# declare-lab/tango

Measured on NVIDIA H100. Metric: audio_seconds_per_second, higher is better.
Workload: dtype bf16

## Files before the change

### tango_b200/csrc/attention_tc.cu

```cuda
#include "tng_ptx.cuh"
#include "tng_internal.h"
#include <stdlib.h>

namespace tng {

constexpr int AT_BM = 128;
constexpr int AT_BN = 64;
constexpr int AT_D = 64;
constexpr int AT_QCHUNK = AT_BM * 128;
constexpr int AT_KCHUNK = AT_BN * 128;
constexpr int AT_NB = 3;
constexpr int AT_THREADS = 256;

struct AttnParams {
  int Lq, Lk, heads;
  int q_col0, q_lo_off, k_col0, k_lo_off, v_col0, v_lo_off;
  const float* kbias;
  __nv_bfloat16* out;
  long long ld_o;
  int split_off;
  float scale_log2e;
};

template <int NSPLIT>
struct AttnCfg {
  static constexpr int Q_BYTES = NSPLIT * AT_QCHUNK;
  static constexpr int KV_BYTES = NSPLIT * AT_KCHUNK;
  static constexpr int SMEM_BYTES = Q_BYTES + AT_NB * 2 * KV_BYTES + 128;
};

template <int NSPLIT>
__global__ void __launch_bounds__(AT_THREADS, (NSPLIT == 1) ? 2 : 1)
attention_kernel(const __grid_constant__ CUtensorMap qmap, const __grid_constant__ CUtensorMap kmap,
                 const __grid_constant__ CUtensorMap vmap, const __grid_constant__ AttnParams p) {
  using Cfg = AttnCfg<NSPLIT>;
  extern __shared__ __align__(1024) uint8_t smem[];
  uint8_t* sQ = smem;
  uint8_t* sK = sQ + Cfg::Q_BYTES;
  uint8_t* sV = sK + AT_NB * Cfg::KV_BYTES;
  uint64_t* bars = reinterpret_cast<uint64_t*>(sV + AT_NB * Cfg::KV_BYTES);
  uint64_t* bar_q = bars;
  uint64_t* full_k = bars + 1;
  uint64_t* full_v = bars + 1 + AT_NB;
  uint64_t* empty_k = bars + 1 + 2 * AT_NB;
  uint64_t* empty_v = bars + 1 + 3 * AT_NB;

  const int tid = threadIdx.x;
  const int warp = tid >> 5;
  const int lane = tid & 31;
  const int wg = warp >> 2;
  const int q0 = blockIdx.x * AT_BM;
  const int head = blockIdx.y;
  const int b = blockIdx.z;
  const int n_tiles = (p.Lk + AT_BN - 1) / AT_BN;

  auto load_k = [&](int t) {
    const int buf = t % AT_NB;
    mbar_arrive_expect_tx(&full_k[buf], Cfg::KV_BYTES);
#pragma unroll
    for (int s = 0; s < NSPLIT; ++s)
      tma_load_3d(sK + buf * Cfg::KV_BYTES + s * AT_KCHUNK, &kmap, &full_k[buf], p.k_col0 + s * p.k_lo_off + head * AT_D,
                  t * AT_BN, b);
  };
  auto load_v = [&](int t) {
    const int buf = t % AT_NB;
    mbar_arrive_expect_tx(&full_v[buf], Cfg::KV_BYTES);
#pragma unroll
    for (int s = 0; s < NSPLIT; ++s)
      tma_load_3d(sV + buf * Cfg::KV_BYTES + s * AT_KCHUNK, &vmap, &full_v[buf], p.v_col0 + s * p.v_lo_off + head * AT_D,
                  t * AT_BN, b);
  };

  if (tid == 0) {
    if ((smem_u32(smem) & 1023u) != 0) __trap();
    tma_prefetch_desc(&qmap);
    tma_prefetch_desc(&kmap);
    tma_prefetch_desc(&vmap);
    mbar_init(bar_q, 1);
    for (int i = 0; i < AT_NB; ++i) {
      mbar_init(&full_k[i], 1);
      mbar_init(&full_v[i], 1);
      mbar_init(&empty_k[i], 2);
      mbar_init(&empty_v[i], 2);
    }
    fence_mbar_init();
    mbar_arrive_expect_tx(bar_q, Cfg::Q_BYTES);
#pragma unroll
    for (int s = 0; s < NSPLIT; ++s)
      tma_load_3d(sQ + s * AT_QCHUNK, &qmap, bar_q, p.q_col0 + s * p.q_lo_off + head * AT_D, q0, b);
    for (int t = 0; t < AT_NB && t < n_tiles; ++t) { load_k(t); load_v(t); }
  }
  __syncthreads();

  constexpr int NT = (NSPLIT == 1) ? 1 : 3;
  const int qsel[3] = {0, 1, 0}, ksel[3] = {0, 0, 1};
  const uint32_t q_base = smem_u32(sQ) + wg * (64 * 128);
  const uint32_t k_base = smem_u32(sK), v_base = smem_u32(sV);
  const float sc = p.scale_log2e;
  constexpr float LOG2E = 1.4426950408889634f;
  const float* kb = p.kbias ? p.kbias + static_cast<long long>(b) * p.Lk : nullptr;
  const int t4 = lane & 3;
  float m_run[2] = {-INFINITY, -INFINITY};
  float l_run[2] = {0.f, 0.f};
  float o[32];
#pragma unroll
  for (int i = 0; i < 32; ++i) o[i] = 0.f;

  mbar_wait(bar_q, 0);
  for (int t = 0; t < n_tiles; ++t) {
    const int buf = t % AT_NB;
    const uint32_t ph = (t / AT_NB) & 1;
    if (tid == 0 && t >= 1 && t - 1 + AT_NB < n_tiles) {
      const int pb = (t - 1) % AT_NB;
      const uint32_t pph = ((t - 1) / AT_NB) & 1;
      mbar_wait(&empty_k[pb], pph);
      load_k(t - 1 + AT_NB);
      mbar_wait(&empty_v[pb], pph);
      load_v(t - 1 + AT_NB);
    }
    float s[32];
    mbar_wait(&full_k[buf], ph);
    fence_regs(s);
    wgmma_fence();
#pragma unroll
    for (int u = 0; u < NT; ++u) {
      const uint64_t qd = wgmma_desc_sw128(q_base + qsel[u] * AT_QCHUNK, 16, 1024);
      const uint64_t kd = wgmma_desc_sw128(k_base + buf * Cfg::KV_BYTES + ksel[u] * AT_KCHUNK, 16, 1024);
#pragma unroll
      for (int k = 0; k < AT_D / 16; ++k) wgmma_ss<64>(s, qd + 2 * k, kd + 2 * k, (u > 0 || k > 0) ? 1u : 0u);
    }
    wgmma_commit();
    wgmma_wait<0>();
    fence_regs(s);
    if ((tid & 127) == 0) mbar_arrive(&empty_k[buf]);

    const int kv0 = t * AT_BN;
    const bool tail = (kb != nullptr) || (kv0 + AT_BN > p.Lk);
#pragma unroll
    for (int j = 0; j < 8; ++j) {
#pragma unroll
      for (int e = 0; e < 2; ++e) {
        float bias = 0.f;
        if (tail) {
          const int kv = kv0 + 8 * j + 2 * t4 + e;
          bias = kv < p.Lk ? (kb ? __ldg(kb + kv) * LOG2E : 0.f) : -INFINITY;
        }
        s[4 * j + e] = fmaf(s[4 * j + e], sc, bias);
        s[4 * j + 2 + e] = fmaf(s[4 * j + 2 + e], sc, bias);
      }
    }
    float corr[2];
    softmax_step(s, m_run, l_run, corr);
    rescale_rows(o, corr);
    uint32_t pa[NSPLIT][4][4];
    pack_p(pa[0], s);
    if constexpr (NSPLIT == 2) pack_p<true>(pa[1], s);

    mbar_wait(&full_v[buf], ph);
    fence_regs(o);
    wgmma_fence();
#pragma unroll
    for (int u = 0; u < NT; ++u) {
      const int ps = (NSPLIT == 2 && u == 1) ? NSPLIT - 1 : 0;
      const uint64_t vd = wgmma_desc_sw128(v_base + buf * Cfg::KV_BYTES + ksel[u] * AT_KCHUNK, 1024, 1024);
#pragma unroll
      for (int kk = 0; kk < AT_BN / 16; ++kk) wgmma_rs_n64_tb(o, pa[ps][kk], vd + ((kk * 2048) >> 4), 1u);
    }
    wgmma_commit();
    wgmma_wait<0>();
    fence_regs(o);
    if ((tid & 127) == 0) mbar_arrive(&empty_v[buf]);
  }

  float inv[2];
  softmax_inv(l_run, inv);
#pragma unroll
  for (int h = 0; h < 2; ++h) {
    const int q = q0 + 64 * wg + 16 * (warp & 3) + (lane >> 2) + 8 * h;
    if (q >= p.Lq) continue;
    __nv_bfloat16* op = p.out + (static_cast<long long>(b) * p.Lq + q) * p.ld_o + head * AT_D + 2 * t4;
#pragma unroll
    for (int j = 0; j < 8; ++j) {
      const float y0 = o[4 * j + 2 * h] * inv[h], y1 = o[4 * j + 2 * h + 1] * inv[h];
      *reinterpret_cast<uint32_t*>(op + 8 * j) = pack_bf16(y0, y1);
      if (p.split_off > 0)
        *reinterpret_cast<uint32_t*>(op + p.split_off + 8 * j) = pack_bf16_lo(y0, y1);
    }
  }
}

template <int NSPLIT>
static int launch_attn(const tng_attn_desc* d, const CUtensorMap& qm, const CUtensorMap& km, const CUtensorMap& vm,
                       const AttnParams& p, cudaStream_t st) {
  const int rc = set_max_dynamic_smem<attention_kernel<NSPLIT>>(AttnCfg<NSPLIT>::SMEM_BYTES, "attention");
  if (rc) return rc;
  dim3 grid((d->Lq + AT_BM - 1) / AT_BM, d->heads, d->batch);
  attention_kernel<NSPLIT><<<grid, AT_THREADS, AttnCfg<NSPLIT>::SMEM_BYTES, st>>>(qm, km, vm, p);
  return check_launch("attention");
}

}

using namespace tng;

extern "C" int tng_attention(const tng_attn_desc* d, void* stream) {
  if (!d || !d->q || !d->k || !d->v || !d->out) return set_error(TNG_EINVAL, "attention: null argument");
  if (d->nsplit != 1 && d->nsplit != 2) return set_error(TNG_EINVAL, "attention: nsplit=%d", d->nsplit);
  if (d->batch <= 0 || d->heads <= 0 || d->Lq <= 0 || d->Lk <= 0) return set_error(TNG_EINVAL, "attention: bad sizes");
  if (d->scale <= 0.f) return set_error(TNG_EINVAL, "attention: scale must be positive");
  if (d->ld_o % 8 || d->split_off % 8 || (reinterpret_cast<uintptr_t>(d->out) & 15))
    return set_error(TNG_EINVAL, "attention: output must allow 16-byte stores");
  AttnParams p;
  p.Lq = d->Lq; p.Lk = d->Lk; p.heads = d->heads;
  p.q_col0 = d->q_col0; p.q_lo_off = d->q_lo_off;
  p.k_col0 = d->k_col0; p.k_lo_off = d->k_lo_off;
  p.v_col0 = d->v_col0; p.v_lo_off = d->v_lo_off;
  p.kbias = d->kbias;
  p.out = reinterpret_cast<__nv_bfloat16*>(d->out);
  p.ld_o = d->ld_o; p.split_off = d->split_off;
  p.scale_log2e = d->scale * 1.4426950408889634f;
  CUtensorMap qm, km, vm;
  int rc = encode_tmap_rows_bf16(&qm, d->q, d->ld_q, d->Lq, d->batch, AT_BM);
  if (!rc) rc = encode_tmap_rows_bf16(&km, d->k, d->ld_k, d->Lk, d->batch, AT_BN);
  if (!rc) rc = encode_tmap_rows_bf16(&vm, d->v, d->ld_v, d->Lk, d->batch, AT_BN);
  if (rc) return rc;
  cudaStream_t st = reinterpret_cast<cudaStream_t>(stream);
  if (d->nsplit == 2) return launch_attn<2>(d, qm, km, vm, p, st);
  return launch_attn<1>(d, qm, km, vm, p, st);
}
```

### tango_b200/csrc/tng_ptx.cuh

```cuda
#pragma once
#include <cuda_runtime.h>
#include <cuda_bf16.h>
#include <cuda.h>
#include <stdint.h>
#include <stdio.h>
#include "../../include/tango_b200.h"

namespace tng {

#ifndef TNG_SPIN_LIMIT
#define TNG_SPIN_LIMIT (1u << 28)
#endif

__device__ __forceinline__ uint32_t smem_u32(const void* p) {
  return static_cast<uint32_t>(__cvta_generic_to_shared(p));
}

__device__ __forceinline__ void mbar_init(uint64_t* bar, uint32_t count) {
  asm volatile("mbarrier.init.shared::cta.b64 [%0], %1;" ::"r"(smem_u32(bar)), "r"(count));
}
__device__ __forceinline__ void fence_mbar_init() {
  asm volatile("fence.mbarrier_init.release.cluster;" ::: "memory");
}
__device__ __forceinline__ void mbar_arrive_expect_tx(uint64_t* bar, uint32_t bytes) {
  asm volatile("mbarrier.arrive.expect_tx.shared::cta.b64 _, [%0], %1;" ::"r"(smem_u32(bar)), "r"(bytes)
               : "memory");
}
__device__ __forceinline__ void mbar_arrive(uint64_t* bar) {
  asm volatile("mbarrier.arrive.shared::cta.b64 _, [%0];" ::"r"(smem_u32(bar)) : "memory");
}
__device__ __forceinline__ void mbar_arrive_if(uint64_t* bar, bool pred) {
  asm volatile(
      "{\n\t.reg .pred p;\n\tsetp.ne.b32 p, %1, 0;\n\t@p mbarrier.arrive.shared::cta.b64 _, [%0];\n\t}"
      ::"r"(smem_u32(bar)), "r"((uint32_t)pred) : "memory");
}
template <int N>
__device__ __forceinline__ void setmaxnreg_dec() { asm volatile("setmaxnreg.dec.sync.aligned.u32 %0;" ::"n"(N)); }
template <int N>
__device__ __forceinline__ void setmaxnreg_inc() { asm volatile("setmaxnreg.inc.sync.aligned.u32 %0;" ::"n"(N)); }
__device__ __forceinline__ uint32_t mbar_try_wait(uint64_t* bar, uint32_t parity) {
  uint32_t ok;
  asm volatile(
      "{\n\t"
      ".reg .pred P;\n\t"
      "mbarrier.try_wait.parity.shared::cta.b64 P, [%1], %2;\n\t"
      "selp.u32 %0, 1, 0, P;\n\t"
      "}\n"
      : "=r"(ok)
      : "r"(smem_u32(bar)), "r"(parity)
      : "memory");
  return ok;
}
__device__ __forceinline__ void mbar_wait(uint64_t* bar, uint32_t parity) {
  uint32_t spins = 0;
  while (!mbar_try_wait(bar, parity)) {
    if (++spins > TNG_SPIN_LIMIT) __trap();
  }
}

__device__ __forceinline__ void tma_prefetch_desc(const CUtensorMap* m) {
  asm volatile("prefetch.tensormap [%0];" ::"l"(reinterpret_cast<uint64_t>(m)) : "memory");
}
__device__ __forceinline__ void tma_load_2d(void* smem, const CUtensorMap* m, uint64_t* bar, int c0, int c1) {
  asm volatile(
      "cp.async.bulk.tensor.2d.shared::cluster.global.mbarrier::complete_tx::bytes [%0], [%1, {%3, %4}], [%2];"
      ::"r"(smem_u32(smem)), "l"(reinterpret_cast<uint64_t>(m)), "r"(smem_u32(bar)), "r"(c0), "r"(c1)
      : "memory");
}
__device__ __forceinline__ void tma_load_3d(void* smem, const CUtensorMap* m, uint64_t* bar, int c0, int c1,
                                            int c2) {
  asm volatile(
      "cp.async.bulk.tensor.3d.shared::cluster.global.mbarrier::complete_tx::bytes [%0], [%1, {%3, %4, %5}], [%2];"
      ::"r"(smem_u32(smem)), "l"(reinterpret_cast<uint64_t>(m)), "r"(smem_u32(bar)), "r"(c0), "r"(c1), "r"(c2)
      : "memory");
}
__device__ __forceinline__ void tma_load_4d(void* smem, const CUtensorMap* m, uint64_t* bar, int c0, int c1,
                                            int c2, int c3) {
  asm volatile(
      "cp.async.bulk.tensor.4d.shared::cluster.global.mbarrier::complete_tx::bytes [%0], [%1, {%3, %4, %5, %6}], "
      "[%2];" ::"r"(smem_u32(smem)),
      "l"(reinterpret_cast<uint64_t>(m)), "r"(smem_u32(bar)), "r"(c0), "r"(c1), "r"(c2), "r"(c3)
      : "memory");
}

__device__ __forceinline__ void wgmma_fence() { asm volatile("wgmma.fence.sync.aligned;" ::: "memory"); }
__device__ __forceinline__ void wgmma_commit() { asm volatile("wgmma.commit_group.sync.aligned;" ::: "memory"); }
template <int N>
__device__ __forceinline__ void wgmma_wait() {
  asm volatile("wgmma.wait_group.sync.aligned %0;" ::"n"(N) : "memory");
}
template <int R>
__device__ __forceinline__ void fence_regs(float (&d)[R]) {
#pragma unroll
  for (int i = 0; i < R; ++i) asm volatile("" : "+f"(d[i])::"memory");
}

__device__ __forceinline__ uint64_t wgmma_desc_sw128(uint32_t saddr, uint32_t lbo_bytes, uint32_t sbo_bytes) {
  uint64_t d = 0;
  d |= static_cast<uint64_t>((saddr & 0x3FFFF) >> 4);
  d |= static_cast<uint64_t>((lbo_bytes >> 4) & 0x3FFF) << 16;
  d |= static_cast<uint64_t>((sbo_bytes >> 4) & 0x3FFF) << 32;
  d |= static_cast<uint64_t>(1) << 62;
  return d;
}

template <int N>
__device__ __forceinline__ void wgmma_ss(float (&d)[N / 2], uint64_t a_desc, uint64_t b_desc, uint32_t scale_d);

template <>
__device__ __forceinline__ void wgmma_ss<32>(float (&d)[16], uint64_t a_desc, uint64_t b_desc, uint32_t scale_d) {
  asm volatile(
      "{\n\t.reg .pred p;\n\tsetp.ne.b32 p, %18, 0;\n\t"
      "wgmma.mma_async.sync.aligned.m64n32k16.f32.bf16.bf16 {%0, %1, %2, %3, %4, %5, %6, %7, %8, %9, %10, %11, %12, %13, %14, %15}, %16, %17, p, 1, 1, 0, 0;\n\t}\n"
      : "+f"(d[0]), "+f"(d[1]), "+f"(d[2]), "+f"(d[3]), "+f"(d[4]), "+f"(d[5]), "+f"(d[6]), "+f"(d[7]),
        "+f"(d[8]), "+f"(d[9]), "+f"(d[10]), "+f"(d[11]), "+f"(d[12]), "+f"(d[13]), "+f"(d[14]), "+f"(d[15])
      : "l"(a_desc), "l"(b_desc), "r"(scale_d));
}

template <>
__device__ __forceinline__ void wgmma_ss<64>(float (&d)[32], uint64_t a_desc, uint64_t b_desc, uint32_t scale_d) {
  asm volatile(
      "{\n\t.reg .pred p;\n\tsetp.ne.b32 p, %34, 0;\n\t"
      "wgmma.mma_async.sync.aligned.m64n64k16.f32.bf16.bf16 {%0, %1, %2, %3, %4, %5, %6, %7, %8, %9, %10, %11, %12, %13, %14, %15, %16, %17, %18, %19, %20, %21, %22, %23, %24, %25, %26, %27, %28, %29, %30, %31}, %32, %33, p, 1, 1, 0, 0;\n\t}\n"
      : "+f"(d[0]), "+f"(d[1]), "+f"(d[2]), "+f"(d[3]), "+f"(d[4]), "+f"(d[5]), "+f"(d[6]), "+f"(d[7]),
        "+f"(d[8]), "+f"(d[9]), "+f"(d[10]), "+f"(d[11]), "+f"(d[12]), "+f"(d[13]), "+f"(d[14]), "+f"(d[15]),
        "+f"(d[16]), "+f"(d[17]), "+f"(d[18]), "+f"(d[19]), "+f"(d[20]), "+f"(d[21]), "+f"(d[22]), "+f"(d[23]),
        "+f"(d[24]), "+f"(d[25]), "+f"(d[26]), "+f"(d[27]), "+f"(d[28]), "+f"(d[29]), "+f"(d[30]), "+f"(d[31])
      : "l"(a_desc), "l"(b_desc), "r"(scale_d));
}

template <>
__device__ __forceinline__ void wgmma_ss<128>(float (&d)[64], uint64_t a_desc, uint64_t b_desc, uint32_t scale_d) {
  asm volatile(
      "{\n\t.reg .pred p;\n\tsetp.ne.b32 p, %66, 0;\n\t"
      "wgmma.mma_async.sync.aligned.m64n128k16.f32.bf16.bf16 {%0, %1, %2, %3, %4, %5, %6, %7, %8, %9, %10, %11, %12, %13, %14, %15, %16, %17, %18, %19, %20, %21, %22, %23, %24, %25, %26, %27, %28, %29, %30, %31, %32, %33, %34, %35, %36, %37, %38, %39, %40, %41, %42, %43, %44, %45, %46, %47, %48, %49, %50, %51, %52, %53, %54, %55, %56, %57, %58, %59, %60, %61, %62, %63}, %64, %65, p, 1, 1, 0, 0;\n\t}\n"
      : "+f"(d[0]), "+f"(d[1]), "+f"(d[2]), "+f"(d[3]), "+f"(d[4]), "+f"(d[5]), "+f"(d[6]), "+f"(d[7]),
        "+f"(d[8]), "+f"(d[9]), "+f"(d[10]), "+f"(d[11]), "+f"(d[12]), "+f"(d[13]), "+f"(d[14]), "+f"(d[15]),
        "+f"(d[16]), "+f"(d[17]), "+f"(d[18]), "+f"(d[19]), "+f"(d[20]), "+f"(d[21]), "+f"(d[22]), "+f"(d[23]),
        "+f"(d[24]), "+f"(d[25]), "+f"(d[26]), "+f"(d[27]), "+f"(d[28]), "+f"(d[29]), "+f"(d[30]), "+f"(d[31]),
        "+f"(d[32]), "+f"(d[33]), "+f"(d[34]), "+f"(d[35]), "+f"(d[36]), "+f"(d[37]), "+f"(d[38]), "+f"(d[39]),
        "+f"(d[40]), "+f"(d[41]), "+f"(d[42]), "+f"(d[43]), "+f"(d[44]), "+f"(d[45]), "+f"(d[46]), "+f"(d[47]),
        "+f"(d[48]), "+f"(d[49]), "+f"(d[50]), "+f"(d[51]), "+f"(d[52]), "+f"(d[53]), "+f"(d[54]), "+f"(d[55]),
        "+f"(d[56]), "+f"(d[57]), "+f"(d[58]), "+f"(d[59]), "+f"(d[60]), "+f"(d[61]), "+f"(d[62]), "+f"(d[63])
      : "l"(a_desc), "l"(b_desc), "r"(scale_d));
}

template <>
__device__ __forceinline__ void wgmma_ss<160>(float (&d)[80], uint64_t a_desc, uint64_t b_desc, uint32_t scale_d) {
  asm volatile(
      "{\n\t.reg .pred p;\n\tsetp.ne.b32 p, %82, 0;\n\t"
      "wgmma.mma_async.sync.aligned.m64n160k16.f32.bf16.bf16 {%0, %1, %2, %3, %4, %5, %6, %7, %8, %9, %10, %11, %12, %13, %14, %15, %16, %17, %18, %19, %20, %21, %22, %23, %24, %25, %26, %27, %28, %29, %30, %31, %32, %33, %34, %35, %36, %37, %38, %39, %40, %41, %42, %43, %44, %45, %46, %47, %48, %49, %50, %51, %52, %53, %54, %55, %56, %57, %58, %59, %60, %61, %62, %63, %64, %65, %66, %67, %68, %69, %70, %71, %72, %73, %74, %75, %76, %77, %78, %79}, %80, %81, p, 1, 1, 0, 0;\n\t}\n"
      : "+f"(d[0]), "+f"(d[1]), "+f"(d[2]), "+f"(d[3]), "+f"(d[4]), "+f"(d[5]), "+f"(d[6]), "+f"(d[7]),
        "+f"(d[8]), "+f"(d[9]), "+f"(d[10]), "+f"(d[11]), "+f"(d[12]), "+f"(d[13]), "+f"(d[14]), "+f"(d[15]),
        "+f"(d[16]), "+f"(d[17]), "+f"(d[18]), "+f"(d[19]), "+f"(d[20]), "+f"(d[21]), "+f"(d[22]), "+f"(d[23]),
        "+f"(d[24]), "+f"(d[25]), "+f"(d[26]), "+f"(d[27]), "+f"(d[28]), "+f"(d[29]), "+f"(d[30]), "+f"(d[31]),
        "+f"(d[32]), "+f"(d[33]), "+f"(d[34]), "+f"(d[35]), "+f"(d[36]), "+f"(d[37]), "+f"(d[38]), "+f"(d[39]),
        "+f"(d[40]), "+f"(d[41]), "+f"(d[42]), "+f"(d[43]), "+f"(d[44]), "+f"(d[45]), "+f"(d[46]), "+f"(d[47]),
        "+f"(d[48]), "+f"(d[49]), "+f"(d[50]), "+f"(d[51]), "+f"(d[52]), "+f"(d[53]), "+f"(d[54]), "+f"(d[55]),
        "+f"(d[56]), "+f"(d[57]), "+f"(d[58]), "+f"(d[59]), "+f"(d[60]), "+f"(d[61]), "+f"(d[62]), "+f"(d[63]),
        "+f"(d[64]), "+f"(d[65]), "+f"(d[66]), "+f"(d[67]), "+f"(d[68]), "+f"(d[69]), "+f"(d[70]), "+f"(d[71]),
        "+f"(d[72]), "+f"(d[73]), "+f"(d[74]), "+f"(d[75]), "+f"(d[76]), "+f"(d[77]), "+f"(d[78]), "+f"(d[79])
      : "l"(a_desc), "l"(b_desc), "r"(scale_d));
}

template <>
__device__ __forceinline__ void wgmma_ss<256>(float (&d)[128], uint64_t a_desc, uint64_t b_desc, uint32_t scale_d) {
  asm volatile(
      "{\n\t.reg .pred p;\n\tsetp.ne.b32 p, %130, 0;\n\t"
      "wgmma.mma_async.sync.aligned.m64n256k16.f32.bf16.bf16 {%0, %1, %2, %3, %4, %5, %6, %7, %8, %9, %10, %11, %12, %13, %14, %15, %16, %17, %18, %19, %20, %21, %22, %23, %24, %25, %26, %27, %28, %29, %30, %31, %32, %33, %34, %35, %36, %37, %38, %39, %40, %41, %42, %43, %44, %45, %46, %47, %48, %49, %50, %51, %52, %53, %54, %55, %56, %57, %58, %59, %60, %61, %62, %63, %64, %65, %66, %67, %68, %69, %70, %71, %72, %73, %74, %75, %76, %77, %78, %79, %80, %81, %82, %83, %84, %85, %86, %87, %88, %89, %90, %91, %92, %93, %94, %95, %96, %97, %98, %99, %100, %101, %102, %103, %104, %105, %106, %107, %108, %109, %110, %111, %112, %113, %114, %115, %116, %117, %118, %119, %120, %121, %122, %123, %124, %125, %126, %127}, %128, %129, p, 1, 1, 0, 0;\n\t}\n"
      : "+f"(d[0]), "+f"(d[1]), "+f"(d[2]), "+f"(d[3]), "+f"(d[4]), "+f"(d[5]), "+f"(d[6]), "+f"(d[7]),
        "+f"(d[8]), "+f"(d[9]), "+f"(d[10]), "+f"(d[11]), "+f"(d[12]), "+f"(d[13]), "+f"(d[14]), "+f"(d[15]),
        "+f"(d[16]), "+f"(d[17]), "+f"(d[18]), "+f"(d[19]), "+f"(d[20]), "+f"(d[21]), "+f"(d[22]), "+f"(d[23]),
        "+f"(d[24]), "+f"(d[25]), "+f"(d[26]), "+f"(d[27]), "+f"(d[28]), "+f"(d[29]), "+f"(d[30]), "+f"(d[31]),
        "+f"(d[32]), "+f"(d[33]), "+f"(d[34]), "+f"(d[35]), "+f"(d[36]), "+f"(d[37]), "+f"(d[38]), "+f"(d[39]),
        "+f"(d[40]), "+f"(d[41]), "+f"(d[42]), "+f"(d[43]), "+f"(d[44]), "+f"(d[45]), "+f"(d[46]), "+f"(d[47]),
        "+f"(d[48]), "+f"(d[49]), "+f"(d[50]), "+f"(d[51]), "+f"(d[52]), "+f"(d[53]), "+f"(d[54]), "+f"(d[55]),
        "+f"(d[56]), "+f"(d[57]), "+f"(d[58]), "+f"(d[59]), "+f"(d[60]), "+f"(d[61]), "+f"(d[62]), "+f"(d[63]),
        "+f"(d[64]), "+f"(d[65]), "+f"(d[66]), "+f"(d[67]), "+f"(d[68]), "+f"(d[69]), "+f"(d[70]), "+f"(d[71]),
        "+f"(d[72]), "+f"(d[73]), "+f"(d[74]), "+f"(d[75]), "+f"(d[76]), "+f"(d[77]), "+f"(d[78]), "+f"(d[79]),
        "+f"(d[80]), "+f"(d[81]), "+f"(d[82]), "+f"(d[83]), "+f"(d[84]), "+f"(d[85]), "+f"(d[86]), "+f"(d[87]),
        "+f"(d[88]), "+f"(d[89]), "+f"(d[90]), "+f"(d[91]), "+f"(d[92]), "+f"(d[93]), "+f"(d[94]), "+f"(d[95]),
        "+f"(d[96]), "+f"(d[97]), "+f"(d[98]), "+f"(d[99]), "+f"(d[100]), "+f"(d[101]), "+f"(d[102]), "+f"(d[103]),
        "+f"(d[104]), "+f"(d[105]), "+f"(d[106]), "+f"(d[107]), "+f"(d[108]), "+f"(d[109]), "+f"(d[110]), "+f"(d[111]),
        "+f"(d[112]), "+f"(d[113]), "+f"(d[114]), "+f"(d[115]), "+f"(d[116]), "+f"(d[117]), "+f"(d[118]), "+f"(d[119]),
        "+f"(d[120]), "+f"(d[121]), "+f"(d[122]), "+f"(d[123]), "+f"(d[124]), "+f"(d[125]), "+f"(d[126]), "+f"(d[127])
      : "l"(a_desc), "l"(b_desc), "r"(scale_d));
}

__device__ __forceinline__ void wgmma_rs_n64_tb(float (&d)[32], const uint32_t (&a)[4], uint64_t b_desc, uint32_t scale_d) {
  asm volatile(
      "{\n\t.reg .pred p;\n\tsetp.ne.b32 p, %37, 0;\n\t"
      "wgmma.mma_async.sync.aligned.m64n64k16.f32.bf16.bf16 {%0, %1, %2, %3, %4, %5, %6, %7, %8, %9, %10, %11, %12, %13, %14, %15, %16, %17, %18, %19, %20, %21, %22, %23, %24, %25, %26, %27, %28, %29, %30, %31}, {%32, %33, %34, %35}, %36, p, 1, 1, 1;\n\t}\n"
      : "+f"(d[0]), "+f"(d[1]), "+f"(d[2]), "+f"(d[3]), "+f"(d[4]), "+f"(d[5]), "+f"(d[6]), "+f"(d[7]),
        "+f"(d[8]), "+f"(d[9]), "+f"(d[10]), "+f"(d[11]), "+f"(d[12]), "+f"(d[13]), "+f"(d[14]), "+f"(d[15]),
        "+f"(d[16]), "+f"(d[17]), "+f"(d[18]), "+f"(d[19]), "+f"(d[20]), "+f"(d[21]), "+f"(d[22]), "+f"(d[23]),
        "+f"(d[24]), "+f"(d[25]), "+f"(d[26]), "+f"(d[27]), "+f"(d[28]), "+f"(d[29]), "+f"(d[30]), "+f"(d[31])
      : "r"(a[0]), "r"(a[1]), "r"(a[2]), "r"(a[3]), "l"(b_desc), "r"(scale_d));
}

__device__ __forceinline__ float ex2_approx(float x) {
  float y;
  asm("ex2.approx.ftz.f32 %0, %1;" : "=f"(y) : "f"(x));
  return y;
}
__device__ __forceinline__ float rcp_approx(float x) {
  float y;
  asm("rcp.approx.ftz.f32 %0, %1;" : "=f"(y) : "f"(x));
  return y;
}
__device__ __forceinline__ float silu_f(float x) {
  return x * rcp_approx(1.0f + ex2_approx(x * -1.4426950408889634f));
}
__device__ __forceinline__ float gelu_erf_f(float x) {
  const float w = fabsf(x) * 0.84932180028801904272f;
  const float t = rcp_approx(fmaf(0.27273748088f, w, 1.0f));
  const float e = ex2_approx(w * -w);
  float poly = fmaf(0.5307027145f, t, -0.7265760135f);
  poly = fmaf(poly, t, 0.7107068705f);
  poly = fmaf(poly, t, -0.142248368f);
  poly = fmaf(poly, t, 0.127414796f);
  const float q = poly * t * e;
  const float phi = x >= 0.0f ? 1.0f - q : q;
  return x * phi;
}
__device__ __forceinline__ float gelu_tanh_f(float x) {
  const float w = x * fmaf(x * x, 0.044715f, 1.0f);
  return x * rcp_approx(1.0f + ex2_approx(w * -2.3022081986f));
}
__device__ __forceinline__ float act_f(float x, int act, float p) {
  if (act == TNG_ACT_SILU) return silu_f(x);
  if (act == TNG_ACT_LRELU) return x > 0.f ? x : x * p;
  return x;
}
__device__ __forceinline__ float warp_sum(float v) {
#pragma unroll
  for (int o = 16; o > 0; o >>= 1) v += __shfl_xor_sync(0xffffffffu, v, o);
  return v;
}
__device__ __forceinline__ float warp_max(float v) {
#pragma unroll
  for (int o = 16; o > 0; o >>= 1) v = fmaxf(v, __shfl_xor_sync(0xffffffffu, v, o));
  return v;
}
__device__ __forceinline__ float quad_sum(float v) {
  v += __shfl_xor_sync(0xffffffffu, v, 1);
  return v + __shfl_xor_sync(0xffffffffu, v, 2);
}
__device__ __forceinline__ float quad_max(float v) {
  v = fmaxf(v, __shfl_xor_sync(0xffffffffu, v, 1));
  return fmaxf(v, __shfl_xor_sync(0xffffffffu, v, 2));
}

__device__ __forceinline__ float bf16_lo(float v) { return v - __bfloat162float(__float2bfloat16_rn(v)); }
__device__ __forceinline__ uint32_t pack_bf16(float a, float b) {
  __nv_bfloat162 v = __floats2bfloat162_rn(a, b);
  return *reinterpret_cast<uint32_t*>(&v);
}
__device__ __forceinline__ uint32_t pack_bf16_lo(float a, float b) { return pack_bf16(bf16_lo(a), bf16_lo(b)); }
__device__ __forceinline__ float4 load_bf16x4(const __nv_bfloat16* p) {
  const uint2 u = *reinterpret_cast<const uint2*>(p);
  const float2 a = __bfloat1622float2(*reinterpret_cast<const __nv_bfloat162*>(&u.x));
  const float2 b = __bfloat1622float2(*reinterpret_cast<const __nv_bfloat162*>(&u.y));
  return make_float4(a.x, a.y, b.x, b.y);
}
__device__ __forceinline__ void store4_bf16(__nv_bfloat16* p, float4 v) {
  uint2 u;
  u.x = pack_bf16(v.x, v.y);
  u.y = pack_bf16(v.z, v.w);
  *reinterpret_cast<uint2*>(p) = u;
}
__device__ __forceinline__ void store4_bf16_lo(__nv_bfloat16* p, float4 v) {
  store4_bf16(p, make_float4(bf16_lo(v.x), bf16_lo(v.y), bf16_lo(v.z), bf16_lo(v.w)));
}
__device__ __forceinline__ void store4_split(__nv_bfloat16* p, float4 v, int split_off) {
  store4_bf16(p, v);
  if (split_off > 0) store4_bf16_lo(p + split_off, v);
}
__device__ __forceinline__ void store_bf16_split(__nv_bfloat16* p, float v, int split_off) {
  const __nv_bfloat16 hi = __float2bfloat16_rn(v);
  *p = hi;
  if (split_off > 0) p[split_off] = __float2bfloat16_rn(v - __bfloat162float(hi));
}

__device__ __forceinline__ void softmax_step(float (&s)[32], float (&m_run)[2], float (&l_run)[2], float (&corr)[2]) {
  float mx[2] = {-INFINITY, -INFINITY};
#pragma unroll
  for (int j = 0; j < 8; ++j) {
#pragma unroll
    for (int e = 0; e < 2; ++e) {
      mx[0] = fmaxf(mx[0], s[4 * j + e]);
      mx[1] = fmaxf(mx[1], s[4 * j + 2 + e]);
    }
  }
  float m_use[2];
#pragma unroll
  for (int h = 0; h < 2; ++h) {
    const float m_new = fmaxf(m_run[h], quad_max(mx[h]));
    m_use[h] = (m_new == -INFINITY) ? 0.f : m_new;
    corr[h] = ex2_approx(m_run[h] - m_use[h]);
    m_run[h] = m_new;
    l_run[h] *= corr[h];
  }
#pragma unroll
  for (int j = 0; j < 8; ++j) {
#pragma unroll
    for (int e = 0; e < 2; ++e) {
      s[4 * j + e] = ex2_approx(s[4 * j + e] - m_use[0]);
      s[4 * j + 2 + e] = ex2_approx(s[4 * j + 2 + e] - m_use[1]);
      l_run[0] += s[4 * j + e];
      l_run[1] += s[4 * j + 2 + e];
    }
  }
}
__device__ __forceinline__ void rescale_rows(float (&o)[32], const float (&corr)[2]) {
#pragma unroll
  for (int j = 0; j < 8; ++j) {
    o[4 * j] *= corr[0]; o[4 * j + 1] *= corr[0];
    o[4 * j + 2] *= corr[1]; o[4 * j + 3] *= corr[1];
  }
}
template <bool LO = false>
__device__ __forceinline__ void pack_p(uint32_t (&pa)[4][4], const float (&s)[32]) {
#pragma unroll
  for (int kk = 0; kk < 4; ++kk)
#pragma unroll
    for (int r = 0; r < 4; ++r) {
      const float x0 = s[8 * kk + 2 * r], x1 = s[8 * kk + 2 * r + 1];
      pa[kk][r] = LO ? pack_bf16_lo(x0, x1) : pack_bf16(x0, x1);
    }
}
__device__ __forceinline__ void softmax_inv(const float (&l_run)[2], float (&inv)[2]) {
#pragma unroll
  for (int h = 0; h < 2; ++h) inv[h] = 1.0f / quad_sum(l_run[h]);
}

}
```

Baseline: 11.92.

## Warp-specialize attention with TMA producer, ping-pong consumers, and software-pipelined softmax

After: 12.26 (median of 6 runs). +2.9%, better.

```diff
diff --git a/tango_b200/csrc/attention_tc.cu b/tango_b200/csrc/attention_tc.cu
--- a/tango_b200/csrc/attention_tc.cu
+++ b/tango_b200/csrc/attention_tc.cu
@@ -5,12 +5,10 @@
 namespace tng {
 
 constexpr int AT_BM = 128;
-constexpr int AT_BN = 64;
 constexpr int AT_D = 64;
 constexpr int AT_QCHUNK = AT_BM * 128;
-constexpr int AT_KCHUNK = AT_BN * 128;
-constexpr int AT_NB = 3;
-constexpr int AT_THREADS = 256;
+constexpr int AT_THREADS = 384;
+constexpr int AT_EX2_FMA_EVERY = 8;
 
 struct AttnParams {
   int Lq, Lk, heads;
@@ -24,26 +22,31 @@
 
 template <int NSPLIT>
 struct AttnCfg {
+  static constexpr int BN = (NSPLIT == 1) ? 128 : 64;
+  static constexpr int STAGES = 3;
+  static constexpr int KCHUNK = BN * 128;
   static constexpr int Q_BYTES = NSPLIT * AT_QCHUNK;
-  static constexpr int KV_BYTES = NSPLIT * AT_KCHUNK;
-  static constexpr int SMEM_BYTES = Q_BYTES + AT_NB * 2 * KV_BYTES + 128;
+  static constexpr int KV_BYTES = NSPLIT * KCHUNK;
+  static constexpr int SMEM_BYTES = Q_BYTES + STAGES * 2 * KV_BYTES + 128;
 };
 
 template <int NSPLIT>
-__global__ void __launch_bounds__(AT_THREADS, (NSPLIT == 1) ? 2 : 1)
+__global__ void __launch_bounds__(AT_THREADS, 1)
 attention_kernel(const __grid_constant__ CUtensorMap qmap, const __grid_constant__ CUtensorMap kmap,
                  const __grid_constant__ CUtensorMap vmap, const __grid_constant__ AttnParams p) {
   using Cfg = AttnCfg<NSPLIT>;
+  constexpr int STAGES = Cfg::STAGES;
+  constexpr int BN = Cfg::BN;
   extern __shared__ __align__(1024) uint8_t smem[];
   uint8_t* sQ = smem;
   uint8_t* sK = sQ + Cfg::Q_BYTES;
-  uint8_t* sV = sK + AT_NB * Cfg::KV_BYTES;
-  uint64_t* bars = reinterpret_cast<uint64_t*>(sV + AT_NB * Cfg::KV_BYTES);
+  uint8_t* sV = sK + STAGES * Cfg::KV_BYTES;
+  uint64_t* bars = reinterpret_cast<uint64_t*>(sV + STAGES * Cfg::KV_BYTES);
   uint64_t* bar_q = bars;
   uint64_t* full_k = bars + 1;
-  uint64_t* full_v = bars + 1 + AT_NB;
-  uint64_t* empty_k = bars + 1 + 2 * AT_NB;
-  uint64_t* empty_v = bars + 1 + 3 * AT_NB;
+  uint64_t* full_v = bars + 1 + STAGES;
+  uint64_t* empty_k = bars + 1 + 2 * STAGES;
+  uint64_t* empty_v = bars + 1 + 3 * STAGES;
 
   const int tid = threadIdx.x;
   const int warp = tid >> 5;
@@ -52,24 +55,7 @@
   const int q0 = blockIdx.x * AT_BM;
   const int head = blockIdx.y;
   const int b = blockIdx.z;
-  const int n_tiles = (p.Lk + AT_BN - 1) / AT_BN;
-
-  auto load_k = [&](int t) {
-    const int buf = t % AT_NB;
-    mbar_arrive_expect_tx(&full_k[buf], Cfg::KV_BYTES);
-#pragma unroll
-    for (int s = 0; s < NSPLIT; ++s)
-      tma_load_3d(sK + buf * Cfg::KV_BYTES + s * AT_KCHUNK, &kmap, &full_k[buf], p.k_col0 + s * p.k_lo_off + head * AT_D,
-                  t * AT_BN, b);
-  };
-  auto load_v = [&](int t) {
-    const int buf = t % AT_NB;
-    mbar_arrive_expect_tx(&full_v[buf], Cfg::KV_BYTES);
-#pragma unroll
-    for (int s = 0; s < NSPLIT; ++s)
-      tma_load_3d(sV + buf * Cfg::KV_BYTES + s * AT_KCHUNK, &vmap, &full_v[buf], p.v_col0 + s * p.v_lo_off + head * AT_D,
-                  t * AT_BN, b);
-  };
+  const int n_tiles = (p.Lk + BN - 1) / BN;
 
   if (tid == 0) {
     if ((smem_u32(smem) & 1023u) != 0) __trap();
@@ -77,18 +63,240 @@
     tma_prefetch_desc(&kmap);
     tma_prefetch_desc(&vmap);
     mbar_init(bar_q, 1);
-    for (int i = 0; i < AT_NB; ++i) {
+    for (int i = 0; i < STAGES; ++i) {
       mbar_init(&full_k[i], 1);
       mbar_init(&full_v[i], 1);
       mbar_init(&empty_k[i], 2);
       mbar_init(&empty_v[i], 2);
     }
     fence_mbar_init();
+  }
+  __syncthreads();
+
+  if (wg == 0) {
+    setmaxnreg_dec<40>();
+    if (tid == 0) {
+      mbar_arrive_expect_tx(bar_q, Cfg::Q_BYTES);
+#pragma unroll
+      for (int s = 0; s < NSPLIT; ++s)
+        tma_load_3d(sQ + s * AT_QCHUNK, &qmap, bar_q, p.q_col0 + s * p.q_lo_off + head * AT_D, q0, b);
+      for (int t = 0; t < n_tiles; ++t) {
+        const int slot = t % STAGES;
+        const uint32_t use = t / STAGES;
+        if (use > 0) mbar_wait(&empty_k[slot], (use - 1) & 1);
+        mbar_arrive_expect_tx(&full_k[slot], Cfg::KV_BYTES);
+#pragma unroll
+        for (int s = 0; s < NSPLIT; ++s)
+          tma_load_3d(sK + slot * Cfg::KV_BYTES + s * Cfg::KCHUNK, &kmap, &full_k[slot],
+                      p.k_col0 + s * p.k_lo_off + head * AT_D, t * BN, b);
+        if (use > 0) mbar_wait(&empty_v[slot], (use - 1) & 1);
+        mbar_arrive_expect_tx(&full_v[slot], Cfg::KV_BYTES);
+#pragma unroll
+        for (int s = 0; s < NSPLIT; ++s)
+          tma_load_3d(sV + slot * Cfg::KV_BYTES + s * Cfg::KCHUNK, &vmap, &full_v[slot],
+                      p.v_col0 + s * p.v_lo_off + head * AT_D, t * BN, b);
+      }
+    }
+    return;
+  }
+  setmaxnreg_inc<232>();
+
+  const int cg = wg - 1;
+  constexpr int NT = (NSPLIT == 1) ? 1 : 3;
+  const int qsel[3] = {0, 1, 0}, ksel[3] = {0, 0, 1};
+  const uint32_t q_base = smem_u32(sQ) + cg * (64 * 128);
+  const uint32_t k_base = smem_u32(sK), v_base = smem_u32(sV);
+  const bool release = (tid & 127) == 0;
+  const float sc = p.scale_log2e;
+  constexpr float LOG2E = 1.4426950408889634f;
+  const float* kb = p.kbias ? p.kbias + static_cast<long long>(b) * p.Lk : nullptr;
+  const int t4 = lane & 3;
+  float m_run[2] = {-INFINITY, -INFINITY};
+  float l_run[2] = {0.f, 0.f};
+  float o[32];
+#pragma unroll
+  for (int i = 0; i < 32; ++i) o[i] = 0.f;
+  float s[BN / 2];
+  uint32_t pa[NSPLIT][BN / 16][4];
+
+  auto issue_s = [&](int t) {
+    const int slot = t % STAGES;
+    mbar_wait(&full_k[slot], (t / STAGES) & 1);
+    fence_regs(s);
+    wgmma_fence();
+#pragma unroll
+    for (int u = 0; u < NT; ++u) {
+      const uint64_t qd = wgmma_desc_sw128(q_base + qsel[u] * AT_QCHUNK, 16, 1024);
+      const uint64_t kd = wgmma_desc_sw128(k_base + slot * Cfg::KV_BYTES + ksel[u] * Cfg::KCHUNK, 16, 1024);
+#pragma unroll
+      for (int k = 0; k < AT_D / 16; ++k) wgmma_ss<BN>(s, qd + 2 * k, kd + 2 * k, (u > 0 || k > 0) ? 1u : 0u);
+    }
+    wgmma_commit();
+  };
+  auto issue_pv = [&](int t) {
+    const int slot = t % STAGES;
+    mbar_wait(&full_v[slot], (t / STAGES) & 1);
+    fence_regs(o);
+    wgmma_fence();
+#pragma unroll
+    for (int u = 0; u < NT; ++u) {
+      const int ps = (NSPLIT == 2 && u == 1) ? NSPLIT - 1 : 0;
+      const uint64_t vd = wgmma_desc_sw128(v_base + slot * Cfg::KV_BYTES + ksel[u] * Cfg::KCHUNK, 1024, 1024);
+#pragma unroll
+      for (int kk = 0; kk < BN / 16; ++kk) wgmma_rs_n64_tb(o, pa[ps][kk], vd + ((kk * 2048) >> 4), 1u);
+    }
+    wgmma_commit();
+  };
+  auto softmax = [&](int t, float (&corr)[2]) {
+    const int kv0 = t * BN;
+    if ((kb != nullptr) || (kv0 + BN > p.Lk)) {
+#pragma unroll
+      for (int j = 0; j < BN / 8; ++j) {
+#pragma unroll
+        for (int e = 0; e < 2; ++e) {
+          const int kv = kv0 + 8 * j + 2 * t4 + e;
+          const float bias = kv < p.Lk ? (kb ? __ldg(kb + kv) * LOG2E : 0.f) : -INFINITY;
+          s[4 * j + e] = fmaf(s[4 * j + e], sc, bias);
+          s[4 * j + 2 + e] = fmaf(s[4 * j + 2 + e], sc, bias);
+        }
+      }
+      softmax_step(s, m_run, l_run, corr);
+    } else {
+      softmax_step<NSPLIT == 1 ? AT_EX2_FMA_EVERY : 0>(s, m_run, l_run, corr, sc);
+    }
+  };
+  auto pack = [&]() {
+    pack_p(pa[0], s);
+    if constexpr (NSPLIT == 2) pack_p<true>(pa[1], s);
+  };
+
+  if (cg == 1) named_bar_arrive(1, 256);
+  mbar_wait(bar_q, 0);
+  float corr[2];
+  named_bar_sync(1 + cg, 256);
+  issue_s(0);
+  named_bar_arrive(2 - cg, 256);
+  wgmma_wait<0>();
+  fence_regs(s);
+  mbar_arrive_if(&empty_k[0], release);
+  softmax(0, corr);
+  pack();
+  for (int t = 1; t < n_tiles; ++t) {
+    named_bar_sync(1 + cg, 256);
+    issue_s(t);
+    issue_pv(t - 1);
+    named_bar_arrive(2 - cg, 256);
+    wgmma_wait<1>();
+    fence_regs(s);
+    mbar_arrive_if(&empty_k[t % STAGES], release);
+    softmax(t, corr);
+    wgmma_wait<0>();
+    fence_regs(o);
+#pragma unroll
+    for (int i = 0; i < NSPLIT; ++i) fence_regs(pa[i]);
+    mbar_arrive_if(&empty_v[(t - 1) % STAGES], release);
+    rescale_rows(o, corr);
+    pack();
+  }
+  named_bar_sync(1 + cg, 256);
+  issue_pv(n_tiles - 1);
+  if (cg == 0) named_bar_arrive(2, 256);
+  wgmma_wait<0>();
+  fence_regs(o);
+#pragma unroll
+  for (int i = 0; i < NSPLIT; ++i) fence_regs(pa[i]);
+  mbar_arrive_if(&empty_v[(n_tiles - 1) % STAGES], release);
+
+  float inv[2];
+  softmax_inv(l_run, inv);
+#pragma unroll
+  for (int h = 0; h < 2; ++h) {
+    const int q = q0 + 64 * cg + 16 * (warp & 3) + (lane >> 2) + 8 * h;
+    if (q >= p.Lq) continue;
+    __nv_bfloat16* op = p.out + (static_cast<long long>(b) * p.Lq + q) * p.ld_o + head * AT_D + 2 * t4;
+#pragma unroll
+    for (int j = 0; j < 8; ++j) {
+      const float y0 = o[4 * j + 2 * h] * inv[h], y1 = o[4 * j + 2 * h + 1] * inv[h];
+      *reinterpret_cast<uint32_t*>(op + 8 * j) = pack_bf16(y0, y1);
+      if (p.split_off > 0)
+        *reinterpret_cast<uint32_t*>(op + p.split_off + 8 * j) = pack_bf16_lo(y0, y1);
+    }
+  }
+}
+
+constexpr int AS_MAX_LK = 256;
+constexpr int AS_BN = 64;
+constexpr int AS_KCHUNK = AS_BN * 128;
+constexpr int AS_NB = 3;
+constexpr int AS_THREADS = 256;
+
+template <int NSPLIT>
+struct AttnShortCfg {
+  static constexpr int Q_BYTES = NSPLIT * AT_QCHUNK;
+  static constexpr int KV_BYTES = NSPLIT * AS_KCHUNK;
+  static constexpr int SMEM_BYTES = Q_BYTES + AS_NB * 2 * KV_BYTES + 128;
+};
+
+template <int NSPLIT>
+__global__ void __launch_bounds__(AS_THREADS, (NSPLIT == 1) ? 2 : 1)
+attention_short_kernel(const __grid_constant__ CUtensorMap qmap, const __grid_constant__ CUtensorMap kmap,
+                 const __grid_constant__ CUtensorMap vmap, const __grid_constant__ AttnParams p) {
+  using Cfg = AttnShortCfg<NSPLIT>;
+  extern __shared__ __align__(1024) uint8_t smem[];
+  uint8_t* sQ = smem;
+  uint8_t* sK = sQ + Cfg::Q_BYTES;
+  uint8_t* sV = sK + AS_NB * Cfg::KV_BYTES;
+  uint64_t* bars = reinterpret_cast<uint64_t*>(sV + AS_NB * Cfg::KV_BYTES);
+  uint64_t* bar_q = bars;
+  uint64_t* full_k = bars + 1;
+  uint64_t* full_v = bars + 1 + AS_NB;
+  uint64_t* empty_k = bars + 1 + 2 * AS_NB;
+  uint64_t* empty_v = bars + 1 + 3 * AS_NB;
+
+  const int tid = threadIdx.x;
+  const int warp = tid >> 5;
+  const int lane = tid & 31;
+  const int wg = warp >> 2;
+  const int q0 = blockIdx.x * AT_BM;
+  const int head = blockIdx.y;
+  const int b = blockIdx.z;
+  const int n_tiles = (p.Lk + AS_BN - 1) / AS_BN;
+
+  auto load_k = [&](int t) {
+    const int buf = t % AS_NB;
+    mbar_arrive_expect_tx(&full_k[buf], Cfg::KV_BYTES);
+#pragma unroll
+    for (int s = 0; s < NSPLIT; ++s)
+      tma_load_3d(sK + buf * Cfg::KV_BYTES + s * AS_KCHUNK, &kmap, &full_k[buf], p.k_col0 + s * p.k_lo_off + head * AT_D,
+                  t * AS_BN, b);
+  };
+  auto load_v = [&](int t) {
+    const int buf = t % AS_NB;
+    mbar_arrive_expect_tx(&full_v[buf], Cfg::KV_BYTES);
+#pragma unroll
+    for (int s = 0; s < NSPLIT; ++s)
+      tma_load_3d(sV + buf * Cfg::KV_BYTES + s * AS_KCHUNK, &vmap, &full_v[buf], p.v_col0 + s * p.v_lo_off + head * AT_D,
+                  t * AS_BN, b);
+  };
+
+  if (tid == 0) {
+    if ((smem_u32(smem) & 1023u) != 0) __trap();
+    tma_prefetch_desc(&qmap);
+    tma_prefetch_desc(&kmap);
+    tma_prefetch_desc(&vmap);
+    mbar_init(bar_q, 1);
+    for (int i = 0; i < AS_NB; ++i) {
+      mbar_init(&full_k[i], 1);
+      mbar_init(&full_v[i], 1);
+      mbar_init(&empty_k[i], 2);
+      mbar_init(&empty_v[i], 2);
+    }
+    fence_mbar_init();
     mbar_arrive_expect_tx(bar_q, Cfg::Q_BYTES);
 #pragma unroll
     for (int s = 0; s < NSPLIT; ++s)
       tma_load_3d(sQ + s * AT_QCHUNK, &qmap, bar_q, p.q_col0 + s * p.q_lo_off + head * AT_D, q0, b);
-    for (int t = 0; t < AT_NB && t < n_tiles; ++t) { load_k(t); load_v(t); }
+    for (int t = 0; t < AS_NB && t < n_tiles; ++t) { load_k(t); load_v(t); }
   }
   __syncthreads();
 
@@ -108,15 +316,15 @@
 
   mbar_wait(bar_q, 0);
   for (int t = 0; t < n_tiles; ++t) {
-    const int buf = t % AT_NB;
-    const uint32_t ph = (t / AT_NB) & 1;
-    if (tid == 0 && t >= 1 && t - 1 + AT_NB < n_tiles) {
-      const int pb = (t - 1) % AT_NB;
-      const uint32_t pph = ((t - 1) / AT_NB) & 1;
+    const int buf = t % AS_NB;
+    const uint32_t ph = (t / AS_NB) & 1;
+    if (tid == 0 && t >= 1 && t - 1 + AS_NB < n_tiles) {
+      const int pb = (t - 1) % AS_NB;
+      const uint32_t pph = ((t - 1) / AS_NB) & 1;
       mbar_wait(&empty_k[pb], pph);
-      load_k(t - 1 + AT_NB);
+      load_k(t - 1 + AS_NB);
       mbar_wait(&empty_v[pb], pph);
-      load_v(t - 1 + AT_NB);
+      load_v(t - 1 + AS_NB);
     }
     float s[32];
     mbar_wait(&full_k[buf], ph);
@@ -125,7 +333,7 @@
 #pragma unroll
     for (int u = 0; u < NT; ++u) {
       const uint64_t qd = wgmma_desc_sw128(q_base + qsel[u] * AT_QCHUNK, 16, 1024);
-      const uint64_t kd = wgmma_desc_sw128(k_base + buf * Cfg::KV_BYTES + ksel[u] * AT_KCHUNK, 16, 1024);
+      const uint64_t kd = wgmma_desc_sw128(k_base + buf * Cfg::KV_BYTES + ksel[u] * AS_KCHUNK, 16, 1024);
 #pragma unroll
       for (int k = 0; k < AT_D / 16; ++k) wgmma_ss<64>(s, qd + 2 * k, kd + 2 * k, (u > 0 || k > 0) ? 1u : 0u);
     }
@@ -134,8 +342,8 @@
     fence_regs(s);
     if ((tid & 127) == 0) mbar_arrive(&empty_k[buf]);
 
-    const int kv0 = t * AT_BN;
-    const bool tail = (kb != nullptr) || (kv0 + AT_BN > p.Lk);
+    const int kv0 = t * AS_BN;
+    const bool tail = (kb != nullptr) || (kv0 + AS_BN > p.Lk);
 #pragma unroll
     for (int j = 0; j < 8; ++j) {
 #pragma unroll
@@ -162,9 +370,9 @@
 #pragma unroll
     for (int u = 0; u < NT; ++u) {
       const int ps = (NSPLIT == 2 && u == 1) ? NSPLIT - 1 : 0;
-      const uint64_t vd = wgmma_desc_sw128(v_base + buf * Cfg::KV_BYTES + ksel[u] * AT_KCHUNK, 1024, 1024);
-#pragma unroll
-      for (int kk = 0; kk < AT_BN / 16; ++kk) wgmma_rs_n64_tb(o, pa[ps][kk], vd + ((kk * 2048) >> 4), 1u);
+      const uint64_t vd = wgmma_desc_sw128(v_base + buf * Cfg::KV_BYTES + ksel[u] * AS_KCHUNK, 1024, 1024);
+#pragma unroll
+      for (int kk = 0; kk < AS_BN / 16; ++kk) wgmma_rs_n64_tb(o, pa[ps][kk], vd + ((kk * 2048) >> 4), 1u);
     }
     wgmma_commit();
     wgmma_wait<0>();
@@ -192,9 +400,15 @@
 template <int NSPLIT>
 static int launch_attn(const tng_attn_desc* d, const CUtensorMap& qm, const CUtensorMap& km, const CUtensorMap& vm,
                        const AttnParams& p, cudaStream_t st) {
+  dim3 grid((d->Lq + AT_BM - 1) / AT_BM, d->heads, d->batch);
+  if (NSPLIT == 1 && d->Lk <= AS_MAX_LK) {
+    const int rc = set_max_dynamic_smem<attention_short_kernel<1>>(AttnShortCfg<1>::SMEM_BYTES, "attention");
+    if (rc) return rc;
+    attention_short_kernel<1><<<grid, AS_THREADS, AttnShortCfg<1>::SMEM_BYTES, st>>>(qm, km, vm, p);
+    return check_launch("attention");
+  }
   const int rc = set_max_dynamic_smem<attention_kernel<NSPLIT>>(AttnCfg<NSPLIT>::SMEM_BYTES, "attention");
   if (rc) return rc;
-  dim3 grid((d->Lq + AT_BM - 1) / AT_BM, d->heads, d->batch);
   attention_kernel<NSPLIT><<<grid, AT_THREADS, AttnCfg<NSPLIT>::SMEM_BYTES, st>>>(qm, km, vm, p);
   return check_launch("attention");
 }
@@ -221,8 +435,9 @@
   p.scale_log2e = d->scale * 1.4426950408889634f;
   CUtensorMap qm, km, vm;
   int rc = encode_tmap_rows_bf16(&qm, d->q, d->ld_q, d->Lq, d->batch, AT_BM);
-  if (!rc) rc = encode_tmap_rows_bf16(&km, d->k, d->ld_k, d->Lk, d->batch, AT_BN);
-  if (!rc) rc = encode_tmap_rows_bf16(&vm, d->v, d->ld_v, d->Lk, d->batch, AT_BN);
+  const uint32_t bn = (d->nsplit == 2) ? AttnCfg<2>::BN : (d->Lk <= AS_MAX_LK) ? AS_BN : AttnCfg<1>::BN;
+  if (!rc) rc = encode_tmap_rows_bf16(&km, d->k, d->ld_k, d->Lk, d->batch, bn);
+  if (!rc) rc = encode_tmap_rows_bf16(&vm, d->v, d->ld_v, d->Lk, d->batch, bn);
   if (rc) return rc;
   cudaStream_t st = reinterpret_cast<cudaStream_t>(stream);
   if (d->nsplit == 2) return launch_attn<2>(d, qm, km, vm, p, st);
diff --git a/tango_b200/csrc/tng_ptx.cuh b/tango_b200/csrc/tng_ptx.cuh
--- a/tango_b200/csrc/tng_ptx.cuh
+++ b/tango_b200/csrc/tng_ptx.cuh
@@ -33,6 +33,12 @@
   asm volatile(
       "{\n\t.reg .pred p;\n\tsetp.ne.b32 p, %1, 0;\n\t@p mbarrier.arrive.shared::cta.b64 _, [%0];\n\t}"
       ::"r"(smem_u32(bar)), "r"((uint32_t)pred) : "memory");
+}
+__device__ __forceinline__ void named_bar_sync(int id, int count) {
+  asm volatile("bar.sync %0, %1;" ::"r"(id), "r"(count) : "memory");
+}
+__device__ __forceinline__ void named_bar_arrive(int id, int count) {
+  asm volatile("bar.arrive %0, %1;" ::"r"(id), "r"(count) : "memory");
 }
 template <int N>
 __device__ __forceinline__ void setmaxnreg_dec() { asm volatile("setmaxnreg.dec.sync.aligned.u32 %0;" ::"n"(N)); }
@@ -93,6 +99,13 @@
 __device__ __forceinline__ void fence_regs(float (&d)[R]) {
 #pragma unroll
   for (int i = 0; i < R; ++i) asm volatile("" : "+f"(d[i])::"memory");
+}
+template <int K>
+__device__ __forceinline__ void fence_regs(uint32_t (&a)[K][4]) {
+#pragma unroll
+  for (int k = 0; k < K; ++k)
+#pragma unroll
+    for (int i = 0; i < 4; ++i) asm volatile("" : "+r"(a[k][i])::"memory");
 }
 
 __device__ __forceinline__ uint64_t wgmma_desc_sw128(uint32_t saddr, uint32_t lbo_bytes, uint32_t sbo_bytes) {
@@ -203,6 +216,16 @@
   asm("ex2.approx.ftz.f32 %0, %1;" : "=f"(y) : "f"(x));
   return y;
 }
+__device__ __forceinline__ float ex2_fma(float x) {
+  x = fmaxf(x, -126.f);
+  const float t = x + 12582912.f;
+  const float f = x - (t - 12582912.f);
+  float p = fmaf(0.009676047f, f, 0.05592212f);
+  p = fmaf(p, f, 0.24022107f);
+  p = fmaf(p, f, 0.69312102f);
+  p = fmaf(p, f, 1.0000001f);
+  return __int_as_float(__float_as_int(p) + (__float_as_int(t) << 23));
+}
 __device__ __forceinline__ float rcp_approx(float x) {
   float y;
   asm("rcp.approx.ftz.f32 %0, %1;" : "=f"(y) : "f"(x));
@@ -282,31 +305,44 @@
   if (split_off > 0) p[split_off] = __float2bfloat16_rn(v - __bfloat162float(hi));
 }
 
-__device__ __forceinline__ void softmax_step(float (&s)[32], float (&m_run)[2], float (&l_run)[2], float (&corr)[2]) {
-  float mx[2] = {-INFINITY, -INFINITY};
-#pragma unroll
-  for (int j = 0; j < 8; ++j) {
+template <int FMA_EVERY = 0, int R>
+__device__ __forceinline__ void softmax_step(float (&s)[R], float (&m_run)[2], float (&l_run)[2], float (&corr)[2],
+                                             float scale = 1.f) {
+  float mx4[2][4];
+#pragma unroll
+  for (int k = 0; k < 4; ++k) mx4[0][k] = mx4[1][k] = -INFINITY;
+#pragma unroll
+  for (int j = 0; j < R / 4; ++j) {
 #pragma unroll
     for (int e = 0; e < 2; ++e) {
-      mx[0] = fmaxf(mx[0], s[4 * j + e]);
-      mx[1] = fmaxf(mx[1], s[4 * j + 2 + e]);
+      const int k = (2 * j + e) & 3;
+      mx4[0][k] = fmaxf(mx4[0][k], s[4 * j + e]);
+      mx4[1][k] = fmaxf(mx4[1][k], s[4 * j + 2 + e]);
     }
   }
+  float mx[2];
+#pragma unroll
+  for (int h = 0; h < 2; ++h) mx[h] = fmaxf(fmaxf(mx4[h][0], mx4[h][1]), fmaxf(mx4[h][2], mx4[h][3]));
   float m_use[2];
 #pragma unroll
   for (int h = 0; h < 2; ++h) {
-    const float m_new = fmaxf(m_run[h], quad_max(mx[h]));
+    const float m_new = fmaxf(m_run[h], quad_max(mx[h]) * scale);
     m_use[h] = (m_new == -INFINITY) ? 0.f : m_new;
     corr[h] = ex2_approx(m_run[h] - m_use[h]);
     m_run[h] = m_new;
     l_run[h] *= corr[h];
   }
 #pragma unroll
-  for (int j = 0; j < 8; ++j) {
+  for (int j = 0; j < R / 4; ++j) {
 #pragma unroll
     for (int e = 0; e < 2; ++e) {
-      s[4 * j + e] = ex2_approx(s[4 * j + e] - m_use[0]);
-      s[4 * j + 2 + e] = ex2_approx(s[4 * j + 2 + e] - m_use[1]);
+      if (FMA_EVERY > 0 && j % FMA_EVERY == FMA_EVERY - 1) {
+        s[4 * j + e] = ex2_fma(fmaf(s[4 * j + e], scale, -m_use[0]));
+        s[4 * j + 2 + e] = ex2_fma(fmaf(s[4 * j + 2 + e], scale, -m_use[1]));
+      } else {
+        s[4 * j + e] = ex2_approx(fmaf(s[4 * j + e], scale, -m_use[0]));
+        s[4 * j + 2 + e] = ex2_approx(fmaf(s[4 * j + 2 + e], scale, -m_use[1]));
+      }
       l_run[0] += s[4 * j + e];
       l_run[1] += s[4 * j + 2 + e];
     }
@@ -319,10 +355,10 @@
     o[4 * j + 2] *= corr[1]; o[4 * j + 3] *= corr[1];
   }
 }
-template <bool LO = false>
-__device__ __forceinline__ void pack_p(uint32_t (&pa)[4][4], const float (&s)[32]) {
-#pragma unroll
-  for (int kk = 0; kk < 4; ++kk)
+template <bool LO = false, int KS>
+__device__ __forceinline__ void pack_p(uint32_t (&pa)[KS][4], const float (&s)[8 * KS]) {
+#pragma unroll
+  for (int kk = 0; kk < KS; ++kk)
 #pragma unroll
     for (int r = 0; r < 4; ++r) {
       const float x0 = s[8 * kk + 2 * r], x1 = s[8 * kk + 2 * r + 1];
```
